# gudgud96/MR-MT3

Hardware: AMD Instinct MI355X
Metric: train segments/sec (T5-small MT3Net, 256-frame mel, 1024-token target; log-mel + fwd + bwd + AdamW) (higher is better)
Workload: dtype bf16; 1 GPU; BASELINE configs[1]: t5 bf16, 64 segments/GPU/step of 32768 samples @16kHz -> 256x512 mel, 1024-token targets, dropout 0.1 on, golden-recipe weights; segments_per_gpu=64, global_segments=64, parallelism=dp1

## Files before the change

### include/mrmt3_hip.h

```cpp
#ifndef MRMT3_HIP_H
#define MRMT3_HIP_H

#include <stddef.h>
#include <stdint.h>

#ifdef __cplusplus
extern "C" {
#endif

#define MRMT3_OK 0
#define MRMT3_ERR_INVALID_ARG 1
#define MRMT3_ERR_HIP 2
#define MRMT3_ERR_UNSUPPORTED 3
#define MRMT3_ERR_COMM 4

#define MRMT3_F32 0
#define MRMT3_BF16 1

int mrmt3_version(void);
const char* mrmt3_last_error(void);
void* mrmt3_host_alloc(size_t bytes);
void mrmt3_host_free(void* p);

#define MRMT3_CNT_GEMM_NT_TILE 0
// ... 145 lines not shown
                    int seq_len, int d, int vocab, int shift, int start_id, int pad_id,
                    int pos_offset, float p_drop, uint64_t seed, const int32_t* step_dev, uint32_t stream_id, void* stream);
size_t mrmt3_embed_bwd_workspace_bytes(int rows, int vocab, int d);
int mrmt3_embed_bwd(const int64_t* ids, const float* dx, float* dtable, int rows, int seq_len, int d,
                    int vocab, int shift, int start_id, int pad_id, float p_drop, uint64_t seed, const int32_t* step_dev,
                    uint32_t stream_id, void* workspace, size_t workspace_bytes, void* stream);
int mrmt3_addpos_fwd(const void* src, int src_dtype, const float* pos, float* x, int rows, int seq_len,
                     int d, int pos_offset, float p_drop, uint64_t seed, const int32_t* step_dev, uint32_t stream_id,
                     void* stream);
int mrmt3_dropmask_cast(const float* dx, void* out, int out_dtype, size_t n, float p_drop, uint64_t seed,
                        const int32_t* step_dev, uint32_t stream_id, void* stream);

int mrmt3_ce_count(const int64_t* targets, int rows, int weighted, int inst_lo, int inst_hi,
                   float* denom_dev, void* stream);
int mrmt3_ce_fwd_bwd(const float* logits, const int64_t* targets, const float* denom_dev,
                     double* loss_dev, void* dlogits, int dl_dtype, int rows, int V, int weighted,
                     int inst_lo, int inst_hi, float grad_scale, void* stream);

int mrmt3_lmhead_ce_fwd_bwd(const void* dec, int ld_dec, const void* W, int ldw, const int64_t* targets,
                            const float* denom_dev, double* loss_dev, void* dlogits, int dl_dtype, int rows, int V,
                            int d, int weighted, int inst_lo, int inst_hi, float grad_scale, void* workspace,
                            size_t workspace_bytes, int chunk_rows, void* stream);

int mrmt3_ce_fwd_bwd_reg(const float* logits, const int64_t* targets, const float* denom_dev, float label_smoothing,
                         float z_loss, double* loss_dev, void* dlogits, int dl_dtype, int rows, int V, int weighted,
                         int inst_lo, int inst_hi, float grad_scale, void* stream);
int mrmt3_lmhead_ce_fwd_bwd_reg(const void* dec, int ld_dec, const void* W, int ldw, const int64_t* targets,
                                const float* denom_dev, float label_smoothing, float z_loss, double* loss_dev,
                                void* dlogits, int dl_dtype, int rows, int V, int d, int weighted, int inst_lo,
                                int inst_hi, float grad_scale, void* workspace, size_t workspace_bytes, int chunk_rows,
                                void* stream);

int mrmt3_token_logprob(const float* logits, const int64_t* targets, float* out, int rows, int V, int ignore_index,
                        void* stream);
int mrmt3_lmhead_logprob(const void* dec, int ld_dec, const void* W, int ldw, const int64_t* targets, float* out,
                         int rows, int V, int d, int dtype, void* workspace, size_t workspace_bytes, int chunk_rows,
                         void* stream);

typedef struct {
  long long begin, end;
  float weight_decay, lr_scale;
} mrmt3_opt_range;
size_t mrmt3_opt_ranges_table_bytes(int n_ranges);
int mrmt3_opt_ranges_plan(const mrmt3_opt_range* ranges, int n_ranges, size_t n, void* table_host, size_t table_bytes,
                          size_t* n_trainable);
int mrmt3_adamw_step(float* p, const float* g, float* m, float* v, float* ema, size_t n, const void* ranges_dev,
                     int n_ranges, size_t n_trainable, const float* lr_dev, int32_t* step_dev, float beta1, float beta2,
                     float eps, float weight_decay, float grad_scale, float ema_decay, const float* stat_dev,
                     float clip_value, void* shadow_bf16, void* stream);
size_t mrmt3_grad_norm_workspace_elems(void);
int mrmt3_grad_norm(const float* g, size_t n, const void* ranges_dev, int n_ranges, float grad_scale, float max_norm,
                    int skip_nonfinite, float* ws, size_t ws_elems, float* stat_dev, int32_t* skipped_dev, void* stream);
int mrmt3_counter_add(int32_t* ctr, int32_t delta, void* stream);
int mrmt3_transpose(const void* in, int in_dtype, void* out, int out_dtype, int rows, int cols,
                    void* stream);
int mrmt3_cast(const void* in, int in_dtype, void* out, int out_dtype, size_t n, void* stream);
int mrmt3_transpose_batched(const void* src_bf16, void* dst_bf16, const void* desc_table,
                            const int* tile_start, int n_mats, int total_tiles, void* stream);

typedef struct mrmt3_decoder mrmt3_decoder;
typedef struct {
  const void* embed;
  const float* pos;
  const void* lm_head;
  const float* final_ln;
  const float* const* ln_self;
  const void* const* w_qkv;
  const void* const* w_o_self;
  const float* const* ln_cross;
  const void* const* w_q_cross;
  const void* const* w_o_cross;
  const float* const* ln_ff;
  const void* const* w_wi;
  const void* const* w_wo;
} mrmt3_decoder_weights;

int mrmt3_decoder_create(mrmt3_decoder** out, int n_layers, int d_model, int n_heads, int d_ff,
                         int vocab, int max_batch, int max_len, int max_enc_len, int w_dtype,
                         float eps);
void mrmt3_decoder_destroy(mrmt3_decoder* dec);
int mrmt3_decoder_begin(mrmt3_decoder* dec, const mrmt3_decoder_weights* w, const void* cross_kv,
                        int batch, int enc_len, int64_t* tokens_out, int start_id, int eos_id,
                        int pad_id, void* stream);
int mrmt3_decoder_set_prefix(mrmt3_decoder* dec, const float* prefix, int n_prefix, void* stream);
int mrmt3_decoder_set_ban(mrmt3_decoder* dec, const uint8_t* banned_mask, void* stream);
int mrmt3_decoder_set_logprobs(mrmt3_decoder* dec, float* out, int ld, void* stream);
int mrmt3_decoder_set_sampling(mrmt3_decoder* dec, float temperature, int top_k, float top_p,
                               unsigned long long seed, void* stream);
int mrmt3_sample_logits(const float* logits, int rows, int V, const uint8_t* banned_mask, float temperature, int top_k,
                        float top_p, unsigned long long seed, int step, int row0, int64_t* tokens_out,
                        float* logp_out, void* stream);
int mrmt3_decoder_begin_beam(mrmt3_decoder* dec, const mrmt3_decoder_weights* w, const void* cross_kv,
                             int groups, int num_beams, int enc_len, int64_t* tokens_out, int start_id,
                             int eos_id, int pad_id, float length_penalty, const uint8_t* banned_mask,
                             int32_t* backptr, float* beam_scores, int32_t* hyps, void* stream);
int mrmt3_decoder_beam_finalize(mrmt3_decoder* dec, int64_t* out_ids, int ld, int max_length, void* stream);
int mrmt3_decoder_beam_finalize_logprobs(mrmt3_decoder* dec, int64_t* out_ids, float* out_logp, int ld,
                                         int max_length, void* stream);
int mrmt3_decoder_run(mrmt3_decoder* dec, int n_steps, void* stream);
int mrmt3_decoder_graph_captured(const mrmt3_decoder* dec);
int mrmt3_decoder_capture_count(const mrmt3_decoder* dec);
int mrmt3_decoder_poll(mrmt3_decoder* dec, int32_t* state_out_pinned, void* stream);
int mrmt3_decoder_logits(mrmt3_decoder* dec, float* dst, int rows, void* stream);

typedef struct {
  int shift0, n_shift;
// ... 42 lines not shown
```

### mr-mt3_amd/csrc/api.hip

```cpp
#include <stdarg.h>
#include <stdio.h>
#include <stdlib.h>

#include <atomic>
#include <mutex>

#include "common.h"

static thread_local char g_err[512] = "";

void mrmt3_set_error(const char* fmt, ...) {
  va_list ap;
  va_start(ap, fmt);
  vsnprintf(g_err, sizeof(g_err), fmt, ap);
  va_end(ap);
}

#ifdef MRMT3_DIAG
int mrmt3_diag_env(const char* name) {
  const char* e = getenv(name);
  const int v = e ? atoi(e) : 0;
  if (v != 0) {
    static std::atomic<unsigned> warned{0};
    const unsigned bit = 1u << ((unsigned char)name[6] & 31);
// ... 19 lines not shown
  *out = (int)v;
  return true;
}
int knob_resolve(const char* name, int dflt) {
  for (int i = 0; i < g_knob_n_over; ++i)
    if (strcmp(g_knob_over[i].name, name) == 0) return g_knob_over[i].value;
  int v;
  return knob_parse(getenv(name), &v) ? v : dflt;
}
}

int mrmt3_knob_get(MrKnob* k, int dflt) {
#ifndef MRMT3_DIAG
  if (__atomic_load_n(&k->state, __ATOMIC_ACQUIRE) == 1) return __atomic_load_n(&k->value, __ATOMIC_RELAXED);
#endif
  std::lock_guard<std::mutex> lock(g_knob_mu);
  const int v = knob_resolve(k->name, dflt);
#ifndef MRMT3_DIAG
  if (!k->registered) { k->registered = 1; k->next = g_knob_sites; g_knob_sites = k; }
  __atomic_store_n(&k->value, v, __ATOMIC_RELAXED);
  __atomic_store_n(&k->state, 1, __ATOMIC_RELEASE);
#endif
  return v;
}

extern "C" int mrmt3_set_knob(const char* name, int value) {
  if (name == nullptr || strncmp(name, "MRMT3_", 6) != 0 || strlen(name) >= sizeof(g_knob_over[0].name)) {
    mrmt3_set_error("set_knob: a knob is named MRMT3_<SWITCH> (at most %zu characters)", sizeof(g_knob_over[0].name) - 1);
    return MRMT3_ERR_INVALID_ARG;
  }
  std::lock_guard<std::mutex> lock(g_knob_mu);
  int i = 0;
  while (i < g_knob_n_over && strcmp(g_knob_over[i].name, name) != 0) ++i;
  if (i == g_knob_n_over) {
    if (g_knob_n_over == (int)(sizeof(g_knob_over) / sizeof(g_knob_over[0]))) {
      mrmt3_set_error("set_knob: more than %d overrides", g_knob_n_over);
      return MRMT3_ERR_INVALID_ARG;
    }
    strcpy(g_knob_over[g_knob_n_over++].name, name);
  }
  g_knob_over[i].value = value;
  for (MrKnob* k = g_knob_sites; k != nullptr; k = k->next)
    if (strcmp(k->name, name) == 0) __atomic_store_n(&k->state, 0, __ATOMIC_RELEASE);
  return MRMT3_OK;
}

extern "C" int mrmt3_reset_knobs(void) {
  std::lock_guard<std::mutex> lock(g_knob_mu);
  g_knob_n_over = 0;
  for (MrKnob* k = g_knob_sites; k != nullptr; k = k->next) __atomic_store_n(&k->state, 0, __ATOMIC_RELEASE);
  return MRMT3_OK;
}

extern "C" int mrmt3_version(void) { return 123;  }
extern "C" const char* mrmt3_last_error(void) { return g_err; }

int mrmt3_cu_count() {
  static int n = 0;
  if (n == 0) {
    int dev = 0;
    hipDeviceProp_t prop;
    if (hipGetDevice(&dev) == hipSuccess && hipGetDeviceProperties(&prop, dev) == hipSuccess) n = prop.multiProcessorCount;
    if (n <= 0) n = 256;
  }
  return n;
}

extern "C" void* mrmt3_host_alloc(size_t bytes) {
  void* p = nullptr;
  if (hipHostMalloc(&p, bytes ? bytes : 1, hipHostMallocDefault) != hipSuccess) {
    (void)hipGetLastError();
    mrmt3_set_error("host_alloc: hipHostMalloc(%zu) failed", bytes);
    return nullptr;
  }
  return p;
}
extern "C" void mrmt3_host_free(void* p) {
  if (p) (void)hipHostFree(p);
}

static std::atomic<unsigned long long> g_counts[MRMT3_CNT_N];
void mrmt3_count(int which) {
  if (which >= 0 && which < MRMT3_CNT_N) g_counts[which].fetch_add(1, std::memory_order_relaxed);
}
extern "C" int mrmt3_dispatch_counts(unsigned long long* out, int n, int reset) {
  if (out == nullptr || n < 0) {
    mrmt3_set_error("dispatch_counts: bad arguments");
    return -1;
  }
  for (int i = 0; i < n && i < MRMT3_CNT_N; ++i)
    out[i] = reset ? g_counts[i].exchange(0, std::memory_order_relaxed) : g_counts[i].load(std::memory_order_relaxed);
  for (int i = MRMT3_CNT_N; i < n; ++i) out[i] = 0;
  return MRMT3_CNT_N;
}

extern "C" int mrmt3_stream_capture_status(void* stream) {
  hipStreamCaptureStatus st = hipStreamCaptureStatusNone;
  const hipError_t e = hipStreamIsCapturing((hipStream_t)stream, &st);
  if (e != hipSuccess) {
    (void)hipGetLastError();
    if (e == hipErrorStreamCaptureInvalidated || e == hipErrorStreamCaptureImplicit) return 2;
    mrmt3_set_error("stream_capture_status: %s", hipGetErrorString(e));
    return MRMT3_ERR_HIP;
  }
  return st == hipStreamCaptureStatusNone ? 0 : st == hipStreamCaptureStatusActive ? 1 : 2;
}

// ... 80 lines not shown
```

### mr-mt3_amd/csrc/rowops.hip

```cpp
#include "common.h"
#include "opt_ranges.h"

#pragma clang fp contract(off)

template <typename T> __device__ __forceinline__ void load4(const T* p, float v[4]);
template <> __device__ __forceinline__ void load4<float>(const float* p, float v[4]) {
  f32x4 t = *(const f32x4*)p;
  v[0] = t.x; v[1] = t.y; v[2] = t.z; v[3] = t.w;
}
template <> __device__ __forceinline__ void load4<bf16_t>(const bf16_t* p, float v[4]) {
  u32x2 t = *(const u32x2*)p;
  v[0] = __uint_as_float(t.x << 16); v[1] = __uint_as_float(t.x & 0xFFFF0000u);
  v[2] = __uint_as_float(t.y << 16); v[3] = __uint_as_float(t.y & 0xFFFF0000u);
}
template <typename T> __device__ __forceinline__ void store4(T* p, const float v[4]);
template <> __device__ __forceinline__ void store4<float>(float* p, const float v[4]) {
  *(f32x4*)p = f32x4{v[0], v[1], v[2], v[3]};
}
template <> __device__ __forceinline__ void store4<bf16_t>(bf16_t* p, const float v[4]) {
  *(u32x2*)p = u32x2{pack_bf2(v[0], v[1]), pack_bf2(v[2], v[3])};
}

template <typename T> __device__ __forceinline__ void load4_nt(const T* p, float v[4]);
template <> __device__ __forceinline__ void load4_nt<float>(const float* p, float v[4]) {
// ... 1124 lines not shown
    coef = stat[1];
  }
  const long long total = tab[nr].start;
  const long long base = (long long)blockIdx.x * OG_CHUNK;
  if (base >= total) return;
  const float lr0 = lr_dev[0];
  const int step = step_dev[0] + 1;
  const double bc1 = 1.0 - pow((double)b1, (double)step);
  const double bc2 = 1.0 - pow((double)b2, (double)step);
  const float bc2_sqrt = (float)sqrt(bc2);
  int r = opt_locate(tab, 0, nr, base);
  float step_size = 0.f, decay = 1.f;
  long long r_start = 0, r_next = 0, r_begin4 = 0;
#pragma unroll 1
  for (int k = 0; k < OG_PER_LANE; ++k) {
    const long long i = base + (long long)k * 256 + threadIdx.x;
    if (i >= total) break;
    if (i >= r_next) {
      r = opt_locate(tab, r, nr, i);
      r_start = tab[r].start;
      r_next = tab[r + 1].start;
      r_begin4 = tab[r].begin4;
      const float lr = lr0 * tab[r].lr_scale;
      step_size = (float)((double)lr / bc1);
      decay = 1.f - lr * tab[r].wd;
    }
    const size_t o = (size_t)(r_begin4 + (i - r_start)) * 4;
    float pv[4], gv[4], mv[4], vv[4];
    load4<float>(p + o, pv);
    load4<float>(g + o, gv);
    load4<float>(m + o, mv);
    load4<float>(v + o, vv);
    adamw_update4<CLIP>(pv, gv, mv, vv, gscale, coef, clip_value, decay, b1, b2, bc2_sqrt, eps, step_size);
    store4<float>(p + o, pv);
    store4<float>(m + o, mv);
    store4<float>(v + o, vv);
    if (shadow) store4<bf16_t>(shadow + o, pv);
    if (EMA) {
      float ev[4];
      load4<float>(ema + o, ev);
#pragma unroll
      for (int e = 0; e < 4; ++e) ev[e] = ev[e] + ema_om * (pv[e] - ev[e]);
      store4<float>(ema + o, ev);
    }
  }
}

__global__ void counter_add_kernel(int32_t* ctr, int32_t delta) { ctr[0] += delta; }

extern "C" int mrmt3_counter_add(int32_t* ctr, int32_t delta, void* stream) {
  MR_CHECK_ARG(ctr, "counter_add: bad args");
  hipLaunchKernelGGL(counter_add_kernel, dim3(1), dim3(1), 0, (hipStream_t)stream, ctr, delta);
  MR_CHECK_LAUNCH("counter_add");
  return MRMT3_OK;
}

extern "C" size_t mrmt3_opt_ranges_table_bytes(int n_ranges) {
  return n_ranges < 0 ? 0 : ((size_t)n_ranges + 1) * sizeof(MrOptRec);
}

extern "C" int mrmt3_opt_ranges_plan(const mrmt3_opt_range* ranges, int n_ranges, size_t n, void* table_host,
                                     size_t table_bytes, size_t* n_trainable) {
  MR_CHECK_ARG(ranges && table_host, "opt_ranges_plan: null pointer");
  MR_CHECK_ARG(n_ranges >= 1 && n_ranges <= MR_OPT_MAX_RANGES, "opt_ranges_plan: %d ranges (1 .. %d: freezing everything leaves nothing to step)",
               n_ranges, MR_OPT_MAX_RANGES);
  MR_CHECK_ARG(n > 0 && n % 4 == 0, "opt_ranges_plan: n = %zu must be a positive multiple of 4", n);
  MR_CHECK_ARG(table_bytes >= mrmt3_opt_ranges_table_bytes(n_ranges), "opt_ranges_plan: the table holds %zu bytes, %zu are needed",
               table_bytes, mrmt3_opt_ranges_table_bytes(n_ranges));
  int bad = 0;
  const char* why = mr_opt_ranges_problem(ranges, n_ranges, n, &bad);
  MR_CHECK_ARG(why[0] == 0, "opt_ranges_plan: range %d [%lld, %lld): %s", bad, ranges[bad].begin, ranges[bad].end, why);
  const size_t tr = mr_opt_ranges_fill(ranges, n_ranges, (MrOptRec*)table_host);
  if (n_trainable) *n_trainable = tr;
  return MRMT3_OK;
}

extern "C" int mrmt3_adamw_step(float* p, const float* g, float* m, float* v, float* ema, size_t n, const void* ranges_dev,
                                int n_ranges, size_t n_trainable, const float* lr_dev, int32_t* step_dev, float beta1,
                                float beta2, float eps, float weight_decay, float grad_scale, float ema_decay,
                                const float* stat_dev, float clip_value, void* shadow_bf16, void* stream) {
  MR_CHECK_ARG(p && g && m && v && lr_dev && step_dev && n % 4 == 0, "adamw_step: bad args");
  MR_CHECK_ARG((ranges_dev != nullptr) == (n_ranges != 0),
               "adamw_step: bad args: ranges_dev and n_ranges come together (NULL and 0: the flat form), got %s and %d ranges",
               ranges_dev ? "a table" : "NULL", n_ranges);
  MR_CHECK_ARG(clip_value >= 0.f, "adamw_step: clip_value = %g is negative (0: no clamp)", (double)clip_value);
  MR_CHECK_ARG(stat_dev || clip_value == 0.f, "adamw_step: clip_value needs stat_dev (the clipped form)");
  MR_CHECK_ARG(ema_decay == 0.f || (ema_decay > 0.f && ema_decay < 1.f), "adamw_step: ema_decay = %g is outside (0, 1)",
               (double)ema_decay);
  MR_CHECK_ARG((ema != nullptr) == (ema_decay != 0.f), "adamw_step: ema_decay = %g %s", (double)ema_decay,
               ema ? "but an ema buffer was given (0 < ema_decay < 1 is needed)" : "needs an ema buffer (null was given)");
  hipStream_t s = (hipStream_t)stream;
  bf16_t* shadow = (bf16_t*)shadow_bf16;
  if (!ranges_dev) {
    MR_CHECK_ARG(!ema, "adamw_step: the flat form keeps no EMA (an ema buffer needs a range table)");
    const dim3 grid(ew_blocks(n / 4)), block(256);
#define AW_LAUNCH(C_)                                                                                                  \
  hipLaunchKernelGGL(adamw_kernel<C_>, grid, block, 0, s, p, g, m, v, n / 4, lr_dev, step_dev, beta1, beta2, eps,       \
                     weight_decay, grad_scale, stat_dev, clip_value, shadow)
    if (stat_dev) AW_LAUNCH(true); else AW_LAUNCH(false);
#undef AW_LAUNCH
  } else {
    MR_CHECK_ARG(n_ranges >= 1 && n_ranges <= MR_OPT_MAX_RANGES, "adamw_step: %d ranges (1 .. %d)", n_ranges, MR_OPT_MAX_RANGES);
    MR_CHECK_ARG(n_trainable > 0 && n_trainable % 4 == 0 && n_trainable <= n,
                 "adamw_step: n_trainable = %zu must be a positive multiple of 4, at most n = %zu", n_trainable, n);
    MR_CHECK_ARG(((uintptr_t)ranges_dev & 7) == 0, "adamw_step: the range table must be 8-byte aligned");
    const size_t groups = n_trainable / 4;
// ... 273 lines not shown
```

### mr-mt3_amd/mrmt3/engine.py

```python
from __future__ import annotations

import os

import torch

from . import lib
from .params import FlatParams
from .synthetic import sinusoid_table


class Tape:

    def __init__(self):
        self.ops = []

    def push(self, **kw):
        self.ops.append(kw)

    def pop(self):
        return self.ops.pop()


class Engine:
    def __init__(self, cfg: dict, flat: FlatParams, variant: str = "t5", segmem_length: int = 64,
                 segmem_num_layers: int = 0, compute_dtype=torch.bfloat16, max_pos: int = 5000):
        self.cfg, self.flat, self.variant = cfg, flat, variant
        self.segmem_length, self.segmem_num_layers = segmem_length, segmem_num_layers
        self.dt = compute_dtype
        self.d, self.H, self.dff, self.V = cfg["d_model"], cfg["num_heads"], cfg["d_ff"], cfg["vocab_size"]
        self.inner = cfg["d_kv"] * self.H
        assert cfg["d_kv"] == 64, "kernels are specialised for d_kv = 64"
        self.eps = cfg["layer_norm_epsilon"]
        self.max_pos = max_pos
        self._pos = None
        self._stream_ctr = 0
        self.seed = 365
        self.step_dev = None
        self.y_dtype = compute_dtype
        self.overlap_wgrad = False
        self.res_grad_dtype = (torch.bfloat16 if compute_dtype == torch.bfloat16 and
                               os.environ.get("MRMT3_RES_GRAD", "bf16") == "bf16" else torch.float32)
        self.head_dtype = "bf16"
        self._wt32 = {}
        self.lo_sites = os.environ.get("MRMT3_ATTN_LO", "all")
        self.norm_dw = lib.NormDwBatch() if os.environ.get("MRMT3_NORM_DW_BATCH", "1") != "0" else None
        self.tn_group = lib.TnGroup() if os.environ.get("MRMT3_TN_GROUP", "1") != "0" else None
        self.fuse_rows = int(os.environ.get("MRMT3_FUSE_ROWS", "6")) if compute_dtype == torch.bfloat16 else 0
        self.fuse_normbwd_max_k = int(os.environ.get("MRMT3_FUSE_NORMBWD_MAXK", "1152"))

    def pos(self, device):
        if self._pos is None or self._pos.device != device:
            self._pos = sinusoid_table(self.max_pos, self.d).to(device).contiguous()
        return self._pos

    def _sid(self):
        self._stream_ctr += 1
        return self._stream_ctr

    def W(self, name):
        return self.flat.W(name, self.dt)

    def ln(self, key):
        return self.flat.master(key)

    def WT(self, name):
        if self.dt == torch.bfloat16:
            return self.flat.WT(name)
        t = self._wt32.get(name)
        if t is None:
            w = self.flat.W(name, torch.float32)
            t = torch.empty(w.shape[1], w.shape[0], device=w.device, dtype=torch.float32)
            lib.transpose(w, t)
            self._wt32[name] = t
        return t

    def wgrad(self, a, b, out):
        if self.flat.is_frozen(out):
            return None
        if a.dtype == torch.float32:
            return lib.gemm_tn_f32(a, b, out, accumulate=True)
        if self.tn_group is not None and self.tn_group.ok(a, b, out):
            return self.tn_group.add(a, b, out, accumulate=True)
        return lib.gemm_tn(a, b, out, accumulate=True)

    def ndw(self, key):
        return None if key in self.flat.frozen else self.flat.grad(key)

    def _embed_bwd(self, *a, **kw):
        if "decoder_embed_tokens.weight" not in self.flat.frozen:
            lib.embed_bwd(*a, **kw)

    def encoder_frozen(self) -> bool:
        return self.flat.all_frozen("encoder.") and "proj.weight" in self.flat.frozen

    def segmem_frozen(self) -> bool:
        f = self.flat
        return (f.all_frozen("segmem_encoder.") and "segmem_proj.weight" in f.frozen and
                "decoder_embed_tokens.weight" in f.frozen)

    def _norm_bwd(self, *a, **kw):
        if self.dt == torch.bfloat16:
            return lib.add_rmsnorm_bwd(*a, defer=self.norm_dw, **kw)
        want_dy = kw.pop("want_dy", True)
        dx1, _ = lib.add_rmsnorm_bwd(*a, defer=self.norm_dw, want_dy=False, **kw)
        if not want_dy:
            return dx1, None
        p = kw.get("p", 0.0)
        if p <= 0.0:
            return dx1, dx1
        return dx1, lib.dropmask_cast(dx1, p=p, seed=kw.get("seed", 0), stream_id=kw.get("stream_y", 0),
                                      step=kw.get("step"), out_dtype=torch.float32)

    def _proj_addnorm(self, x, pend, w_norm, xn_dtype=None, **kw):
        xn_dtype = xn_dtype or self.dt
        if pend is None:
            return lib.add_rmsnorm_fwd(x, None, w_norm, self.eps, xn_dtype, **kw)
        a, w = pend
        if ((self.fuse_rows & 1) and self.y_dtype == torch.bfloat16 and xn_dtype == torch.bfloat16 and x.shape[1] == 512 and
                lib.gemm_rows_ok(a, w)):
            return lib.gemm_nt_addnorm(a, w, x, w_norm, self.eps, **kw)
        y = lib.gemm_nt(a, w, out_dtype=self.y_dtype)
        return lib.add_rmsnorm_fwd(x, y, w_norm, self.eps, xn_dtype, **kw)

    def _proj_norm_bwd(self, a, wt, dres, x1, rstd, w_norm, dw, **kw):
        if ((self.fuse_rows & 2) and self.norm_dw is not None and self.y_dtype == torch.bfloat16 and dres is not None and
                x1.shape[1] == 512 and a.shape[1] <= self.fuse_normbwd_max_k and lib.gemm_rows_ok(a, wt)):
            return lib.gemm_nt_normbwd(a, wt, dres, x1, rstd, w_norm, dw, defer=self.norm_dw, **kw)
        dxn = lib.gemm_nt(a, wt, out_dtype=self.y_dtype)
        return self._norm_bwd(dxn, dres, x1, rstd, w_norm, dw, **kw)

    def _proj_geglu_bwd(self, dy, wt, h, **kw):
        if (self.fuse_rows & 4) and h.dtype == torch.bfloat16 and lib.gemm_rows_ok(dy, wt, N=wt.shape[0]):
            return lib.gemm_nt_geglubwd(dy, wt, h, **kw)
        dg = lib.gemm_nt(dy, wt)
        return lib.geglu_bwd(h, dg, **kw)

# ... 417 lines not shown
```

### mr-mt3_amd/mrmt3/lib.py

```python
from __future__ import annotations

import ctypes as C
import os
import re
import subprocess

import torch

F32, BF16 = 0, 1
_HERE = os.path.dirname(os.path.abspath(__file__))
LIB_PATH = os.environ.get("MRMT3_TOOL_LIB") or os.path.join(_HERE, "libmrmt3_hip.so")
HEADER_PATH = os.path.join(os.path.dirname(os.path.dirname(_HERE)), "include", "mrmt3_hip.h")
CSRC_DIR = os.path.join(os.path.dirname(_HERE), "csrc")
_lib = None

vp = C.c_void_p


def _header_text(path: str) -> str:
    return re.sub(r"/\*.*?\*/", "", open(path).read(), flags=re.S)


def header_symbols(path: str = HEADER_PATH):
    return sorted(set(re.findall(r"\b(mrmt3_[a-z0-9_]+)\s*\(", _header_text(path))))
# ... 18 lines not shown
    raise TypeError(f"{what}: no ctypes mapping for the C type '{decl.strip()}'")


def header_signatures(path: str = HEADER_PATH) -> dict:
    sigs = {}
    for ret, name, params in re.findall(r"([\w \t\*]+?)\b(mrmt3_[a-z0-9_]+)\s*\(([^()]*)\)\s*;", _header_text(path)):
        args = []
        for prm in ([] if params.strip() == "void" else params.split(",")):
            m = re.fullmatch(r"\s*(.*?[\s\*])\w+\s*", prm, flags=re.S)
            if m is None:
                raise TypeError(f"{name}: cannot parse the parameter '{prm.strip()}'")
            args.append(_ctype(m.group(1), name))
        sigs[name] = (_ctype(ret, name), args)
    if set(sigs) != set(header_symbols(path)):
        raise TypeError("unparsed prototypes: %s" % sorted(set(sigs) ^ set(header_symbols(path))))
    return sigs


_SIGS = header_signatures()


def build(verbose: bool = False, diag: bool = True) -> str:
    for target in (["all"], ["diag"]) if diag else (["all"],):
        r = subprocess.run(["make", "-C", CSRC_DIR, "-j8"] + target, capture_output=True, text=True)
        if verbose or r.returncode != 0:
            print(r.stdout[-4000:], r.stderr[-4000:])
        if r.returncode != 0:
            raise RuntimeError("building libmrmt3_hip.so failed (make %s)" % target[0])
    return LIB_PATH


def load():
    global _lib
    if _lib is not None:
        return _lib
    if not os.path.exists(LIB_PATH):
        raise RuntimeError(
            f"{LIB_PATH} is missing: the MI355X kernels are the only implementation of this path "
            "(no CPU fallback). Run `python __graft_entry__.py` / `make -C mr-mt3_amd/csrc` first.")
    lib = C.CDLL(LIB_PATH)
    for name, (res, args) in _SIGS.items():
        if os.environ.get("MRMT3_TOOL_LIB") and not hasattr(lib, name):
            continue
        fn = getattr(lib, name)
        fn.restype = res
        fn.argtypes = args
    if not os.environ.get("MRMT3_TOOL_LIB") and lib.mrmt3_version() < MIN_VERSION:
        raise RuntimeError(f"{LIB_PATH} is version {lib.mrmt3_version()}, this binding needs >= {MIN_VERSION}: "
                           "a stale build — run `make -C mr-mt3_amd/csrc`")
    _lib = lib
    return lib


MIN_VERSION = 123
COUNTER_NAMES = ("gemm_nt_tile", "gemm_nt8", "gemm_nt_geglu", "tn_group", "tn8", "tn_tile", "attn_fwd", "attn_bwd",
                 "attn_bwd_onepass", "attn_f32", "tn_f32", "gemm_nt_splitk", "gemm_nt_addnorm", "gemm_nt_normbwd",
                 "gemm_nt_geglubwd", "attn_fwd_varlen", "attn_bwd_varlen", "logmel_wave", "logmel_general")


def set_knob(name: str, value: int):
    _check(load().mrmt3_set_knob(name.encode(), int(value)), "set_knob")


def reset_knobs():
    _check(load().mrmt3_reset_knobs(), "reset_knobs")


def dispatch_counts(reset: bool = False) -> dict:
    arr = (C.c_ulonglong * len(COUNTER_NAMES))()
    n = load().mrmt3_dispatch_counts(arr, len(COUNTER_NAMES), int(reset))
    assert n == len(COUNTER_NAMES), "lib.COUNTER_NAMES is out of step with MRMT3_CNT_N"
    return {k: int(arr[i]) for i, k in enumerate(COUNTER_NAMES)}


PROFILE = None
PROFILE_BYTES = {}


class _Timed:
    def __init__(self, family, work, unit, executed=None):
        self.args = (family, work, unit)
        self.executed = executed

    def __enter__(self):
        if PROFILE is not None:
            self.e0 = torch.cuda.Event(enable_timing=True)
            self.e1 = torch.cuda.Event(enable_timing=True)
            self.e0.record()
        return self

    def __exit__(self, *exc):
        if PROFILE is not None:
            self.e1.record()
            PROFILE.append(self.args + (self.e0, self.e1))
            if self.executed is not None:
                PROFILE.append((self.args[0] + "@executed", self.executed, self.args[2], self.e0, self.e1))
        return False


def _check(rc: int, what: str):
    if rc != 0:
        raise RuntimeError(f"{what} failed (code {rc}): {load().mrmt3_last_error().decode()}")


def _p(t):
    return None if t is None else C.c_void_p(t.data_ptr())

# ... 817 lines not shown
        nbytes = int(L.mrmt3_opt_ranges_table_bytes(len(self.ranges)))
        self.host = torch.zeros(max(nbytes, 8), dtype=torch.uint8)
        tr = C.c_size_t(0)
        rc = L.mrmt3_opt_ranges_plan(arr, len(self.ranges), self.n, C.c_void_p(self.host.data_ptr()), nbytes, C.byref(tr))
        if rc != 0:
            raise ValueError(L.mrmt3_last_error().decode())
        self.n_trainable = int(tr.value)
        self.table = None

    def __len__(self):
        return len(self.ranges)

    def to(self, device):
        if self.table is None or self.table.device != torch.device(device):
            self.table = self.host.to(device)
        return self


def adamw_step(p, g, m, v, lr_dev, step_dev, beta1=0.9, beta2=0.999, eps=1e-8, weight_decay=None, grad_scale=1.0,
               shadow=None, stat=None, clip_value=0.0, ranges: OptRanges = None, ema=None, ema_decay=0.0):
    if ranges is not None and weight_decay is not None:
        raise ValueError("adamw_step: weight_decay comes from the range table; do not pass it together with `ranges`")
    _dev(p, g, m, v, lr_dev, step_dev, stat, ema, None if ranges is None else ranges.table)
    assert stat is None or (stat.dtype == torch.float32 and stat.numel() >= 3)
    assert ranges is None or (p.dtype == torch.float32 and p.is_contiguous() and p.numel() == ranges.n)
    tab, nr, ntr = (None, 0, 0) if ranges is None else (ranges.table, len(ranges), ranges.n_trainable)
    wd = 0.01 if weight_decay is None else weight_decay
    _check(load().mrmt3_adamw_step(_p(p), _p(g), _p(m), _p(v), _p(ema), p.numel(), _p(tab), nr, ntr, _p(lr_dev),
                                   _p(step_dev), beta1, beta2, eps, wd, grad_scale, float(ema_decay), _p(stat),
                                   float(clip_value), _p(shadow), _stream()), "adamw_step")


def grad_norm_workspace(device) -> torch.Tensor:
    return torch.empty(int(load().mrmt3_grad_norm_workspace_elems()), device=device, dtype=torch.float32)


def grad_norm(g, grad_scale, max_norm, skip_nonfinite, ws, stat, skipped, ranges: OptRanges = None):
    _dev(g, ws, stat, skipped, None if ranges is None else ranges.table)
    assert g.dtype == torch.float32 and g.is_contiguous() and ws.dtype == torch.float32
    assert stat.dtype == torch.float32 and stat.numel() >= 3 and skipped.dtype == torch.int32 and skipped.numel() >= 1
    assert ranges is None or g.numel() == ranges.n
    tab, nr = (None, 0) if ranges is None else (ranges.table, len(ranges))
    _check(load().mrmt3_grad_norm(_p(g), g.numel(), _p(tab), nr, float(grad_scale), float(max_norm),
                                  int(bool(skip_nonfinite)), _p(ws), ws.numel(), _p(stat), _p(skipped), _stream()),
           "grad_norm")


def counter_add(ctr, delta=1):
    _dev(ctr)
    assert ctr.dtype == torch.int32 and ctr.numel() >= 1
    _check(load().mrmt3_counter_add(_p(ctr), int(delta), _stream()), "counter_add")


def transpose(src, out):
    _dev(src, out)
    rows, cols = src.shape
    _check(load().mrmt3_transpose(_p(src), _dt(src), _p(out), _dt(out), rows, cols, _stream()), "transpose")
    return out


def cast(src, out):
    _dev(src, out)
    _check(load().mrmt3_cast(_p(src), _dt(src), _p(out), _dt(out), src.numel(), _stream()), "cast")
    return out


def transpose_batched(src_flat, dst_flat, desc_table, tile_start, n_mats, total_tiles):
    _dev(src_flat, dst_flat, desc_table, tile_start)
    _check(load().mrmt3_transpose_batched(_p(src_flat), _p(dst_flat), _p(desc_table), _p(tile_start), n_mats,
                                          total_tiles, _stream()), "transpose_batched")


COMM_ID_BYTES = 128


class Comm:

    def __init__(self, uid: bytes, rank: int, world: int):
        assert len(uid) == COMM_ID_BYTES
        self.rank, self.world = rank, world
        self._h = vp()
        buf = C.create_string_buffer(uid, COMM_ID_BYTES)
        _check(load().mrmt3_comm_create(buf, rank, world, C.byref(self._h)), "comm_create")
        import weakref
        self._fin = weakref.finalize(self, Comm._destroy, self._h)

    @staticmethod
    def _destroy(h):
        if h:
            load().mrmt3_comm_destroy(h)

    def __enter__(self):
        return self

    def __exit__(self, *exc):
        self.close()
        return False

    @staticmethod
    def unique_id() -> bytes:
        buf = C.create_string_buffer(COMM_ID_BYTES)
        _check(load().mrmt3_comm_unique_id(buf), "comm_unique_id")
        return buf.raw

    def allreduce(self, t: torch.Tensor, average: bool = False, stream=None):
        _dev(t)
# ... 73 lines not shown
```

### mr-mt3_amd/mrmt3/trainer.py

```python
from __future__ import annotations

import contextlib
import os

import torch
import torch.distributed as dist

from . import lib
from .ddp import GradBuckets
from .params import ALIASES, ParamGroups, ema_decay_option


_RETIRED = []


def _retire(graph) -> None:
    import ctypes
    _RETIRED.append(graph)
    ctypes.pythonapi.Py_IncRef(ctypes.py_object(graph))


def _first_line(e) -> str:
    t = str(e)
    return t.splitlines()[0] if t else ""
# ... 36 lines not shown
        self._ema_swapped = False
        self.loss_reg, self.label_smoothing, self.z_loss = lib.ce_options(label_smoothing, z_loss)
        self.clip_on, self._max_norm, self._clip_value, self.skip_nonfinite = clip_options(
            gradient_clip_val, gradient_clip_algorithm, skip_nonfinite, track_grad_norm)
        n_acc = int(accumulate_grad_batches)
        if n_acc < 1 or n_acc != accumulate_grad_batches:
            raise ValueError("accumulate_grad_batches must be an integer >= 1, got %r" % (accumulate_grad_batches,))
        self.accumulate = n_acc
        self._micro = 0
        if pack_targets is None:
            pack_targets = os.environ.get("MRMT3_PACK_TARGETS", "0") != "0"
        self.pack_targets = bool(pack_targets)
        if self.pack_targets and model.engine.variant == "segmem_v1":
            raise ValueError("pack_targets is not supported for segmem_v1: its memory slots are prepended to the decoder input, "
                             "so the decoder rows cannot be cut to the scored prefix")
        self.model, self.flat, self.engine = model, model.flat, model.engine
        self.groups = ParamGroups(model.flat.shapes, frozen, no_decay, lr_scale)
        assert model.device.type == "cuda", "the trainer drives the HIP kernels: move the model to the GPU first"
        self.base_lr, self.lr_lambda = lr, lr_lambda
        self.betas, self.eps, self.wd = betas, eps, weight_decay
        self.weighted = weighted_loss
        dev = model.device
        self.lr_dev = torch.full((1,), lr, device=dev, dtype=torch.float32)
        self.step_dev = torch.zeros(1, device=dev, dtype=torch.int32)
        self.host_step = 0
        self.world = dist.get_world_size() if dist.is_available() and dist.is_initialized() else 1
        cfg = model.cfg
        if grad_exchange_dtype is None and os.environ.get("MRMT3_GRAD_EXCHANGE", "f32") == "bf16":
            grad_exchange_dtype = torch.bfloat16
        layers_per_bucket = max(1, int(os.environ.get("MRMT3_DDP_LAYERS_PER_BUCKET", layers_per_bucket)))
        self.buckets = GradBuckets(self.flat, cfg["num_layers"], cfg["num_decoder_layers"],
                                   model.segmem_num_layers > 0, layers_per_bucket, exchange_dtype=grad_exchange_dtype)
        self.buckets.before_fire = model.engine.join_wgrad
        self.flat.ensure_grads()
        self.flat.ensure_adam()
        if self.world > 1:
            dist.broadcast(self.flat.P, src=0)
        self._install_groups()
        if self.ema_decay is not None:
            self.flat.E = None
            self.flat.ensure_ema()
        self.last_loss = None
        self.last_nll = None
        self._clip_stat = self._skipped_dev = self._clip_ws = None
        if self.clip_on:
            self._clip_stat = torch.zeros(4, device=dev, dtype=torch.float32)
            self._skipped_dev = torch.zeros(1, device=dev, dtype=torch.int32)
            self._clip_ws = lib.grad_norm_workspace(dev)
        self.salt_dev = self.step_dev if n_acc == 1 else torch.zeros(1, device=dev, dtype=torch.int32)
        self.engine.step_dev = self.salt_dev
        self.use_graph = (os.environ.get("MRMT3_TRAIN_GRAPH", "1") != "0") if graph is None else bool(graph)
        self._collective_stream_checked = False
        self.graph_warmup = 2
        self._graphs = {}
        self._eager_seen = {}
        self._cap_stream = None
        self._cap_owner = None
        self.pack_graphs = max(1, int(os.environ.get("MRMT3_PACK_GRAPHS", "4")))
        self._pack_lru = []

    def mel_from_audio(self, audio):
        from contrib import spectrograms as sp
        return sp.logmel_segments(audio, out_bf16=(self.engine.dt == torch.bfloat16))

    def _pack_plan(self, labels, tcap):
        if tcap is None:
            return None
        cfg = self.model.cfg
        return lib.pack_plan(labels.contiguous(), tcap, cfg["decoder_start_token_id"], cfg["pad_token_id"])

    def pack_capacity(self, labels):
        if not self.pack_targets:
            return None
        from . import packing
        B, L = labels.shape
        if labels.is_cuda:
            lengths = lib.pack_lengths(labels.contiguous()).cpu().numpy()
        else:
            lengths = packing.row_lengths(labels.numpy())
        tcap = packing.capacity(lengths, B, L)
        return None if tcap == B * L else tcap

    def _phase(self):
        if self.accumulate == 1:
            return None
        if self._micro == 0:
            return "first"
        return "last" if self._micro == self.accumulate - 1 else "middle"

    def _step_body(self, inputs, labels, targets_prev, audio, cut=None, tcap=None, phase=None):
        eng, flat = self.engine, self.flat
        eng.reset_deferred()
        eng._stream_ctr = 0
        mel = self.mel_from_audio(inputs) if audio else inputs
        plan = self._pack_plan(labels, tcap)
        targets = labels.reshape(-1) if plan is None else plan.targets
        if eng.dt == torch.bfloat16:
            dec, tape = eng.forward(mel, labels, targets_prev, training=True, need_grad=True, want_logits=False, pack=plan)
            loss, dl, nll = lib.lmhead_cross_entropy(dec, eng.W("lm_head"), targets, want_grad=True,
                                                     grad_dtype=torch.bfloat16, weighted=self.weighted,
                                                     label_smoothing=self.label_smoothing, z_loss=self.z_loss,
                                                     return_nll=True)
        else:
            logits, tape = eng.forward(mel, labels, targets_prev, training=True, need_grad=True, pack=plan)
            loss, dl, nll = lib.cross_entropy(logits.reshape(-1, logits.shape[-1]), targets, want_grad=True,
                                              grad_dtype=torch.float32, weighted=self.weighted,
                                              label_smoothing=self.label_smoothing, z_loss=self.z_loss, return_nll=True)
        if phase in (None, "first"):
            flat.G.zero_()
        self.buckets.reset()
        if phase in ("first", "middle"):
            eng.backward(tape, dl)
        elif cut is None:
            eng.backward(tape, dl, on_layer_done=self.buckets.on_layer_done)
            self.buckets.finish()
        else:
            sent = set()

            def layer_done(prefix, i):
                idx = [j for j in self.buckets.triggered_by(prefix, i) if j not in sent]
                if idx:
                    sent.update(idx)
                    eng.join_wgrad()
                    cut(idx)
            active = self.buckets.active
            eng.backward(tape, dl, on_layer_done=layer_done if active else None)
            cut([j for j in range(len(self.buckets.buckets)) if j not in sent] if active else [])
        if phase in (None, "last"):
            self._optimizer_tail()
        if self.accumulate > 1:
            lib.counter_add(self.salt_dev, 1)
        return loss, nll

    @property
    def groups_on(self) -> bool:
        return self.flat.opt_ranges is not None

    def _install_groups(self):
        if self.groups.trivial:
            self.flat.set_groups(None, self.wd)
            if self.ema_decay is not None:
                self.flat.all_range(self.wd)
            self.buckets.set_trainable(None)
        else:
            self.flat.set_groups(self.groups, self.wd)
            self.buckets.set_trainable(self.flat.trainable_spans() if self.groups.frozen else None)

    def _drop_graphs(self):
        import gc
        torch.cuda.synchronize()
        self._graphs.clear()
        self._eager_seen.clear()
        self._pack_lru.clear()
        gc.collect()
        torch.cuda.synchronize()

    def set_frozen(self, patterns):
        if self._micro:
            raise RuntimeError("set_frozen: %d micro-batch(es) of an accumulation cycle are pending" % self._micro)
        if self._ema_swapped:
            raise RuntimeError("set_frozen inside `with trainer.ema_weights()`")
        groups = ParamGroups(self.flat.shapes, patterns, self.groups.patterns["no_decay"], self.groups.patterns["lr_scale"])
        self._drop_graphs()
        self.engine.reset_deferred()
        self.groups = groups
        self._install_groups()

    def ema_state_dict(self):
        if self.ema_decay is None:
            raise RuntimeError("ema_state_dict: the trainer was built without ema_decay")
        torch.cuda.current_stream().synchronize()
        out = type(self.model.state_dict())()
        for k, v in self.model.state_dict().items():
            key = ALIASES.get(k, k)
            src = self.flat.view(self.flat.E, key) if key in self.flat.shapes else v
            out[k] = src.detach().cpu().clone()
        return out

    @contextlib.contextmanager
    def ema_weights(self):
        if self.ema_decay is None:
            raise RuntimeError("ema_weights: the trainer was built without ema_decay")
        if self._ema_swapped:
            raise RuntimeError("ema_weights: already inside the context")
        flat = self.flat
        with torch.no_grad():
            keep_p = flat.P.clone()
            keep_s = None if flat.S is None else flat.S.clone()
            flat.P.copy_(flat.E)
            if flat.S is not None:
                flat.refresh_shadows(force=True, need_transposed=flat.ST is not None)
        self._ema_swapped = True
        try:
            yield self
        finally:
            with torch.no_grad():
                flat.P.copy_(keep_p)
                if keep_s is not None:
                    flat.S.copy_(keep_s)
                    if flat.ST is not None:
                        flat.refresh_transposed()
                    flat._shadow_version = flat.master_version()
                else:
                    flat._shadow_version = -1
# ... 369 lines not shown
```

Before: 2594 segments/s.

## Overwrite weight gradients on first write instead of zeroing whole grad buffer

On the first step for a given shape key, the trainer records which weight-gradient GEMMs write their flat-buffer slice exactly once. On later steps it zeroes only the complement ranges with a new multi-range zero kernel, and those wgrad GEMMs run with accumulate disabled. This removes a full memset of the fp32 gradient buffer and the read half of the read-modify-write in the first wgrad GEMM per slice. In exchange it adds record/overwrite bookkeeping with runtime consistency checks, plus a flush of the grouped TN batch when an ungrouped GEMM targets a pending output.

```diff
diff --git a/include/mrmt3_hip.h b/include/mrmt3_hip.h
--- a/include/mrmt3_hip.h
+++ b/include/mrmt3_hip.h
@@ -221,6 +221,7 @@
 int mrmt3_grad_norm(const float* g, size_t n, const void* ranges_dev, int n_ranges, float grad_scale, float max_norm,
                     int skip_nonfinite, float* ws, size_t ws_elems, float* stat_dev, int32_t* skipped_dev, void* stream);
 int mrmt3_counter_add(int32_t* ctr, int32_t delta, void* stream);
+int mrmt3_zero_ranges(float* base, const int64_t* off, const int64_t* len, int n_ranges, size_t max_len, void* stream);
 int mrmt3_transpose(const void* in, int in_dtype, void* out, int out_dtype, int rows, int cols,
                     void* stream);
 int mrmt3_cast(const void* in, int in_dtype, void* out, int out_dtype, size_t n, void* stream);
diff --git a/mr-mt3_amd/csrc/api.hip b/mr-mt3_amd/csrc/api.hip
--- a/mr-mt3_amd/csrc/api.hip
+++ b/mr-mt3_amd/csrc/api.hip
@@ -95,7 +95,7 @@
   return MRMT3_OK;
 }
 
-extern "C" int mrmt3_version(void) { return 123;  }
+extern "C" int mrmt3_version(void) { return 124;  }
 extern "C" const char* mrmt3_last_error(void) { return g_err; }
 
 int mrmt3_cu_count() {
diff --git a/mr-mt3_amd/csrc/rowops.hip b/mr-mt3_amd/csrc/rowops.hip
--- a/mr-mt3_amd/csrc/rowops.hip
+++ b/mr-mt3_amd/csrc/rowops.hip
@@ -1200,6 +1200,30 @@
   MR_CHECK_ARG(ctr, "counter_add: bad args");
   hipLaunchKernelGGL(counter_add_kernel, dim3(1), dim3(1), 0, (hipStream_t)stream, ctr, delta);
   MR_CHECK_LAUNCH("counter_add");
+  return MRMT3_OK;
+}
+
+__global__ __launch_bounds__(256) void zero_ranges_kernel(float* __restrict__ base, const int64_t* __restrict__ off,
+                                                           const int64_t* __restrict__ len) {
+  float* p = base + off[blockIdx.y];
+  const int64_t n = len[blockIdx.y];
+  const int64_t head = min(n, (int64_t)((4 - (((uintptr_t)p >> 2) & 3)) & 3));
+  const int64_t n4 = (n - head) >> 2;
+  const int64_t t = (int64_t)blockIdx.x * blockDim.x + threadIdx.x, T = (int64_t)gridDim.x * blockDim.x;
+  f32x4* p4 = (f32x4*)(p + head);
+  for (int64_t i = t; i < n4; i += T) p4[i] = f32x4{0.f, 0.f, 0.f, 0.f};
+  if (t < head) p[t] = 0.f;
+  const int64_t tail0 = head + 4 * n4;
+  if (t < n - tail0) p[tail0 + t] = 0.f;
+}
+
+extern "C" int mrmt3_zero_ranges(float* base, const int64_t* off, const int64_t* len, int n_ranges, size_t max_len,
+                                 void* stream) {
+  MR_CHECK_ARG(base && off && len && n_ranges > 0 && n_ranges <= 65535 && max_len > 0, "zero_ranges: bad args");
+  const size_t want = (max_len / 4 + 255) / 256;
+  const unsigned gx = (unsigned)(want < 1 ? 1 : (want > 256 ? 256 : want));
+  hipLaunchKernelGGL(zero_ranges_kernel, dim3(gx, (unsigned)n_ranges), dim3(256), 0, (hipStream_t)stream, base, off, len);
+  MR_CHECK_LAUNCH("zero_ranges");
   return MRMT3_OK;
 }
 
diff --git a/mr-mt3_amd/mrmt3/engine.py b/mr-mt3_amd/mrmt3/engine.py
--- a/mr-mt3_amd/mrmt3/engine.py
+++ b/mr-mt3_amd/mrmt3/engine.py
@@ -45,6 +45,10 @@
         self.lo_sites = os.environ.get("MRMT3_ATTN_LO", "all")
         self.norm_dw = lib.NormDwBatch() if os.environ.get("MRMT3_NORM_DW_BATCH", "1") != "0" else None
         self.tn_group = lib.TnGroup() if os.environ.get("MRMT3_TN_GROUP", "1") != "0" else None
+        self._g_mode = None
+        self._g_seen = {}
+        self._g_plan = frozenset()
+        self._g_done = set()
         self.fuse_rows = int(os.environ.get("MRMT3_FUSE_ROWS", "6")) if compute_dtype == torch.bfloat16 else 0
         self.fuse_normbwd_max_k = int(os.environ.get("MRMT3_FUSE_NORMBWD_MAXK", "1152"))
 
@@ -77,11 +81,56 @@
     def wgrad(self, a, b, out):
         if self.flat.is_frozen(out):
             return None
-        if a.dtype == torch.float32:
+        bf16 = a.dtype != torch.float32
+        first_writes = self._g_note(out, bf16) if self._g_mode is not None else False
+        if not bf16:
             return lib.gemm_tn_f32(a, b, out, accumulate=True)
         if self.tn_group is not None and self.tn_group.ok(a, b, out):
-            return self.tn_group.add(a, b, out, accumulate=True)
-        return lib.gemm_tn(a, b, out, accumulate=True)
+            return self.tn_group.add(a, b, out, accumulate=not first_writes)
+        if self.tn_group is not None and any(o.data_ptr() == out.data_ptr() for _, _, o, _ in self.tn_group._sites):
+            self.tn_group.flush()
+        return lib.gemm_tn(a, b, out, accumulate=not first_writes)
+
+    def _g_note(self, out, can_write):
+        key = (out.data_ptr(), out.numel())
+        if self._g_mode == "record":
+            self._g_seen.setdefault(key, bool(can_write and out.is_contiguous()))
+            return False
+        if can_write and key in self._g_plan and key not in self._g_done:
+            self._g_done.add(key)
+            return True
+        if key not in self._g_done and any(key[0] < k[0] + 4 * k[1] and k[0] < key[0] + 4 * key[1] for k in self._g_plan):
+            raise RuntimeError("a weight gradient that the step's plan overwrites was produced through another path first: "
+                               "the step does not launch what its first run with these shapes launched")
+        return False
+
+    def begin_grad_record(self):
+        self._g_mode, self._g_seen = "record", {}
+
+    def end_grad_record(self):
+        seen, self._g_mode, self._g_seen = self._g_seen, None, {}
+        g0 = self.flat.G.data_ptr()
+        spans = sorted((p, p + 4 * n) for p, n in seen)
+        plan = []
+        for (p, n), first_can_write in seen.items():
+            alone = sum(1 for a, b in spans if a < p + 4 * n and p < b) == 1
+            if first_can_write and alone and g0 <= p and p + 4 * n <= g0 + 4 * self.flat.G.numel():
+                plan.append(((p - g0) // 4, n))
+        return tuple(sorted(plan))
+
+    def begin_grad_overwrite(self, plan):
+        g0 = self.flat.G.data_ptr()
+        self._g_mode, self._g_plan, self._g_done = "overwrite", frozenset((g0 + 4 * o, n) for o, n in plan), set()
+
+    def end_grad_overwrite(self):
+        missing = len(self._g_plan) - len(self._g_done)
+        self._g_mode, self._g_plan, self._g_done = None, frozenset(), set()
+        if missing:
+            raise RuntimeError("%d weight gradient(s) the step's plan overwrites were not produced: the step does not "
+                               "launch what its first run with these shapes launched" % missing)
+
+    def abandon_grad_plan(self):
+        self._g_mode, self._g_seen, self._g_plan, self._g_done = None, {}, frozenset(), set()
 
     def ndw(self, key):
         return None if key in self.flat.frozen else self.flat.grad(key)
diff --git a/mr-mt3_amd/mrmt3/lib.py b/mr-mt3_amd/mrmt3/lib.py
--- a/mr-mt3_amd/mrmt3/lib.py
+++ b/mr-mt3_amd/mrmt3/lib.py
@@ -94,7 +94,7 @@
     return lib
 
 
-MIN_VERSION = 123
+MIN_VERSION = 124
 COUNTER_NAMES = ("gemm_nt_tile", "gemm_nt8", "gemm_nt_geglu", "tn_group", "tn8", "tn_tile", "attn_fwd", "attn_bwd",
                  "attn_bwd_onepass", "attn_f32", "tn_f32", "gemm_nt_splitk", "gemm_nt_addnorm", "gemm_nt_normbwd",
                  "gemm_nt_geglubwd", "attn_fwd_varlen", "attn_bwd_varlen", "logmel_wave", "logmel_general")
@@ -1018,6 +1018,12 @@
     _check(load().mrmt3_counter_add(_p(ctr), int(delta), _stream()), "counter_add")
 
 
+def zero_ranges(base, off, length, max_len):
+    _dev(base, off, length)
+    assert base.dtype == torch.float32 and off.dtype == length.dtype == torch.int64 and off.numel() == length.numel() > 0
+    _check(load().mrmt3_zero_ranges(_p(base), _p(off), _p(length), off.numel(), int(max_len), _stream()), "zero_ranges")
+
+
 def transpose(src, out):
     _dev(src, out)
     rows, cols = src.shape
diff --git a/mr-mt3_amd/mrmt3/trainer.py b/mr-mt3_amd/mrmt3/trainer.py
--- a/mr-mt3_amd/mrmt3/trainer.py
+++ b/mr-mt3_amd/mrmt3/trainer.py
@@ -112,6 +112,8 @@
         self.use_graph = (os.environ.get("MRMT3_TRAIN_GRAPH", "1") != "0") if graph is None else bool(graph)
         self._collective_stream_checked = False
         self.graph_warmup = 2
+        self.grad_overwrite = os.environ.get("MRMT3_GRAD_OVERWRITE", "1") != "0"
+        self._g_plans = {}
         self._graphs = {}
         self._eager_seen = {}
         self._cap_stream = None
@@ -140,6 +142,21 @@
             lengths = packing.row_lengths(labels.numpy())
         tcap = packing.capacity(lengths, B, L)
         return None if tcap == B * L else tcap
+
+    def _complement_of(self, plan):
+        gaps, pos = [], 0
+        for o, n in plan:
+            if o > pos:
+                gaps.append((pos, o - pos))
+            pos = max(pos, o + n)
+        if pos < self.flat.G.numel():
+            gaps.append((pos, self.flat.G.numel() - pos))
+        if not plan:
+            return None
+        dev = self.flat.G.device
+        i64 = lambda v: torch.tensor(v, dtype=torch.int64, device=dev)
+        return dict(plan=plan, off=i64([g[0] for g in gaps]) if gaps else None,
+                    len=i64([g[1] for g in gaps]) if gaps else None, max_len=max([g[1] for g in gaps], default=0))
 
     def _phase(self):
         if self.accumulate == 1:
@@ -166,8 +183,21 @@
             loss, dl, nll = lib.cross_entropy(logits.reshape(-1, logits.shape[-1]), targets, want_grad=True,
                                               grad_dtype=torch.float32, weighted=self.weighted,
                                               label_smoothing=self.label_smoothing, z_loss=self.z_loss, return_nll=True)
+        eng.abandon_grad_plan()
+        g_plan = None
         if phase in (None, "first"):
-            flat.G.zero_()
+            g_key = (bool(audio), tuple(mel.shape), tuple(labels.shape),
+                     None if targets_prev is None else tuple(targets_prev.shape), tcap, phase,
+                     eng.dt, eng.tn_group is not None, flat.G.data_ptr())
+            g_plan = self._g_plans.get(g_key) if self.grad_overwrite else None
+            if g_plan is None:
+                flat.G.zero_()
+                if self.grad_overwrite and not torch.cuda.is_current_stream_capturing():
+                    eng.begin_grad_record()
+            else:
+                if g_plan["off"] is not None:
+                    lib.zero_ranges(flat.G, g_plan["off"], g_plan["len"], g_plan["max_len"])
+                eng.begin_grad_overwrite(g_plan["plan"])
         self.buckets.reset()
         if phase in ("first", "middle"):
             eng.backward(tape, dl)
@@ -186,6 +216,11 @@
             active = self.buckets.active
             eng.backward(tape, dl, on_layer_done=layer_done if active else None)
             cut([j for j in range(len(self.buckets.buckets)) if j not in sent] if active else [])
+        if phase in (None, "first"):
+            if g_plan is not None:
+                eng.end_grad_overwrite()
+            elif eng._g_mode == "record":
+                self._g_plans[g_key] = self._complement_of(eng.end_grad_record())
         if phase in (None, "last"):
             self._optimizer_tail()
         if self.accumulate > 1:
@@ -210,6 +245,7 @@
         import gc
         torch.cuda.synchronize()
         self._graphs.clear()
+        self._g_plans.clear()
         self._eager_seen.clear()
         self._pack_lru.clear()
         gc.collect()
```

New measurement: 2598 segments/s (median of 5 runs). Within noise of the previous version (+0.2%).
